# DaDaMrX/ReaLiSe

Measured on AMD Instinct MI355X. Metric: train sentences/sec (seq_len=128), higher is better.
Workload: dtype bf16

## Files before the change

### include/realise_hip_debug.h

```cpp
#ifndef REALISE_HIP_DEBUG_H
#define REALISE_HIP_DEBUG_H
#include "realise_hip.h"
#ifdef __cplusplus
extern "C" {
#endif

void realise_set_tn_transpose_read(int enable);
void realise_set_nt_allow_n96(int on);
void realise_set_nt_variant(int v);
void realise_set_engine(int key, int value);
int realise_gemm_nt_rows(void* stream, int dtype, const void* A, int64_t lda, const void* B, int64_t ldb, int M, int N, int K,
                         const realise_epilogue* ep, const int* rows_dev);
int realise_gemm_nt_live(void* stream, const void* A, int64_t lda, const void* B, int64_t ldb, int M, int N, int K,
                         const realise_epilogue* ep, const int* live_list, const int* live_count);
int realise_gemm_nt_live_rows(void* stream, const void* A, int64_t lda, const void* B, int64_t ldb, int M, int N, int K,
                              const realise_epilogue* ep, const int* row_list, const int* row_count);
int realise_gemm_nt_splitk(void* stream, const void* A, int64_t lda, const void* B, int64_t ldb, int M, int N, int K, int nsplit,
                           float* slab, int64_t slab_stride, const int* m_dev);
int realise_gemm_tn_grouped_live(void* stream, int dtype, int n, const realise_tn_problem* problems, int P, const int* live,
                                 const int* n_live, int list_rows, int overwrite);
int realise_layernorm_bwd_ex(void* stream, const void* dy, const void* xhat, const float* rstd, const float* gamma, void* dx, void* dx_drop,
                             uint32_t drop_seed, uint32_t drop_thresh, float drop_scale, float* dgamma, float* dbeta, float* slots, int rows, int H);
int realise_layernorm_fwd_live(void* stream, const void* x, const float* gamma, const float* beta, float eps, void* y, void* xhat, float* rstd,
                               const uint8_t* row_live, int rows, int H);
int realise_layernorm_bwd_live(void* stream, const void* dy, const void* xhat, const float* rstd, const float* gamma, void* dx, void* dx_drop,
                               uint32_t drop_seed, uint32_t drop_thresh, float drop_scale, float* dgamma, float* dbeta, float* slots,
                               const uint8_t* row_live, int rows, int H);
void realise_set_ln(int key, int value);
int realise_batchnorm_stats_ex(void* stream, const void* x, int P, int C, int hw, const float* counts, int n_stat, const float* gamma, const float* beta,
                               float eps, float momentum, float* running_mean, float* running_var, int64_t* num_batches_tracked, float* mean, float* rstd,
                               float* scale, float* shift, float* sq_scratch, float* slots);
int realise_batchnorm_bwd_ex(void* stream, const void* dy, const void* relu_src, int P, int C, int hw, const float* counts, int n_stat,
                             const void* xa, const float* mean_a, const float* rstd_a, const float* gamma_a, void* dxa, float* dgamma_a, float* dbeta_a,
                             const void* xb, const float* mean_b, const float* rstd_b, const float* gamma_b, void* dxb, float* dgamma_b, float* dbeta_b,
                             float* sums, float* slots);
void realise_set_nt8p(int key, int value);
void realise_set_nt_group_m(int g);
void realise_set_tn_split(int n);
void realise_set_conv_c64(int on);
void realise_set_glyph_dedup(int on);
void realise_set_wgrad_overlap(int on);
void realise_set_branch_overlap(int on);
void realise_set_dgrad_parity(int on);
void realise_set_wgrad_group(int on);

int realise_profile_enable(int max_launches);
void realise_profile_mode(int attached);
void realise_profile_disable(void);
void realise_profile_pause(int paused);
int realise_profile_read(int kernel_family, long long* count, double* total_ms, double* total_work);
int realise_profile_dump(int kernel_family, int max_records, float* ms_out, double* work_out);
// ... 46 lines not shown
```

### realise_amd/_capi.py

```python
import ctypes as C
import os

from .config import MODEL_TYPES

HERE = os.path.dirname(os.path.abspath(__file__))
LIB_PATH = os.path.join(HERE, "librealise_hip.so")

F32, BF16 = 0, 1
F32_BF16X3 = 2
EPI_STORE, EPI_GELU, EPI_DROP_RESID, EPI_GELU_BWD = 0, 1, 2, 4


class GruStep(C.Structure):
    _fields_ = [("n_alive", C.c_int32), ("H", C.c_int32), ("Tp", C.c_int32), ("t", C.c_int32),
                ("table", C.c_void_p), ("pho_idx", C.c_void_p), ("perm", C.c_void_p), ("lens", C.c_void_p),
                ("gh", C.c_void_p), ("b_hh", C.c_void_p), ("h_prev", C.c_void_p), ("h_new", C.c_void_p), ("rzn", C.c_void_p), ("out", C.c_void_p),
                ("dout", C.c_void_p), ("dh", C.c_void_p), ("dgi", C.c_void_p), ("dgh", C.c_void_p), ("onehot", C.c_void_p)]


class Gate(C.Structure):
    _fields_ = [("B", C.c_int32), ("S", C.c_int32), ("H", C.c_int32),
                ("bert", C.c_void_p), ("pho", C.c_void_p), ("res", C.c_void_p), ("masks", C.c_void_p), ("W", C.c_void_p), ("bias", C.c_void_p),
                ("mean", C.c_void_p), ("msum", C.c_void_p), ("g", C.c_void_p), ("fused", C.c_void_p),
                ("dfused", C.c_void_p), ("dbert", C.c_void_p), ("dpho", C.c_void_p), ("dres", C.c_void_p), ("dz", C.c_void_p), ("dW", C.c_void_p),
# ... 68 lines not shown
    "realise_gemm_nt_live": (_I, [_P, _P, _L, _P, _L, _I, _I, _I, C.POINTER(Epilogue), _P, _P]),
    "realise_gemm_nt_live_rows": (_I, [_P, _P, _L, _P, _L, _I, _I, _I, C.POINTER(Epilogue), _P, _P]),
    "realise_gemm_nt_splitk": (_I, [_P, _P, _L, _P, _L, _I, _I, _I, _I, _P, _L, _P]),
    "realise_gemm_tn_grouped_live": (_I, [_P, _I, _I, C.POINTER(TnProblem), _I, _P, _P, _I, _I]),
    "realise_conv_tn": (_I, [_P, _I, _P, _L, C.POINTER(ConvGeom), _I, _I, _I, _P, _P, _L]),
    "realise_set_tn_transpose_read": (None, [_I]),
    "realise_set_nt_allow_n96": (None, [_I]),
    "realise_set_nt_variant": (None, [_I]),
    "realise_set_nt_group_m": (None, [_I]),
    "realise_set_nt8p": (None, [_I, _I]),
    "realise_set_ln": (None, [_I, _I]),
    "realise_set_engine": (None, [_I, _I]),
    "realise_layernorm_bwd_ex": (_I, [_P, _P, _P, _P, _P, _P, _P, C.c_uint32, C.c_uint32, C.c_float, _P, _P, _P, _I, _I]),
    "realise_layernorm_fwd_live": (_I, [_P, _P, _P, _P, C.c_float, _P, _P, _P, _P, _I, _I]),
    "realise_layernorm_bwd_live": (_I, [_P, _P, _P, _P, _P, _P, _P, C.c_uint32, C.c_uint32, C.c_float, _P, _P, _P, _P, _I, _I]),
    "realise_batchnorm_stats_ex": (_I, [_P, _P, _I, _I, _I, _P, _I, _P, _P, C.c_float, C.c_float] + [_P] * 9),
    "realise_batchnorm_bwd_ex": (_I, [_P, _P, _P, _I, _I, _I, _P, _I] + [_P] * 7 + [_P] * 7 + [_P, _P]),
    "realise_debug_bn_plan": (_I, [_I, _I, _I, _I, _I, _I, C.POINTER(BnPlan)]),
    "realise_debug_conv_nt_path": (_I, [_I, C.POINTER(ConvGeom), _L, _I, _I, _I, _I, _I, _I, _I, _L, _L]),
    "realise_conv_nt_ex": (_I, [_P, _I, C.POINTER(ConvGeom), _P, _L, _I, _I, _I, C.POINTER(Epilogue), _P, _I, _P, _L]),
    "realise_conv_dgrad_s2_ex": (_I, [_P, _I, C.POINTER(ConvGeom), _P, _L, _I, C.POINTER(Epilogue), _P]),
    "realise_gemm_nt_ex": (_I, [_P, _I, _P, _L, _P, _L, _I, _I, _I, C.POINTER(Epilogue), _P, _I, _P]),
    "realise_batchnorm_stats_rows": (_I, [_P, _I, _P, _I, _I, _I, _P, _P, _I, _I, _P, _P, _F, _F] + [_P] * 9),
    "realise_batchnorm_apply_rows": (_I, [_P, _I] + [_P] * 7 + [_I, _I, _I, _I, _P]),
    "realise_batchnorm_bwd_rows": (_I, [_P, _I, _P, _P, _I, _I, _I, _P, _P, _I] + [_P] * 7 + [_P] * 7 + [_P, _P]),
    "realise_set_tn_split": (None, [_I]),
    "realise_set_conv_c64": (None, [_I]),
    "realise_set_branch_overlap": (None, [_I]),
    "realise_set_glyph_dedup": (None, [_I]),
    "realise_set_wgrad_overlap": (None, [_I]),
    "realise_set_wgrad_group": (None, [_I]),
    "realise_set_dgrad_parity": (None, [_I]),
    "realise_attention_fwd": (_I, [_P, _I, _P, _P, _P, _L, _P, _P, _L, _P, _I, _I, _I, _U, _U, _F]),
    "realise_attention_bwd": (_I, [_P, _I, _P, _P, _P, _L, _P, _P, _P, _L, _P, _P, _P, _P, _P, _L, _I, _I, _I, _U, _U, _F]),
    "realise_mask_to_additive": (_I, [_P, _P, _P, _I]),
    "realise_layernorm_fwd": (_I, [_P, _I, _P, _P, _P, _F, _P, _P, _P, _I, _I]),
    "realise_layernorm_bwd": (_I, [_P, _I, _P, _P, _P, _P, _P, _P, _P, _I, _I]),
    "realise_layernorm_gelu_bwd": (_I, [_P, _I, _P, _P, _P, _P, _P, _P, _P, _P, _I, _I, _P, _P, _I]),
    "realise_masked_ce": (_I, [_P, _I, _P, _L, _P, _P, _I, _I, _P, _P, _P]),
    "realise_gru_step_fwd": (_I, [_P, _I, C.POINTER(GruStep)]),
    "realise_gru_step_bwd": (_I, [_P, _I, C.POINTER(GruStep)]),
    "realise_gate_fwd": (_I, [_P, _I, C.POINTER(Gate)]),
    "realise_gate_bwd": (_I, [_P, _I, C.POINTER(Gate)]),
    "realise_gate_softmax_fwd": (_I, [_P, _I, C.POINTER(Gate)]),
    "realise_gate_softmax_bwd": (_I, [_P, _I, C.POINTER(Gate)]),
    "realise_sum_fuse_fwd": (_I, [_P, _I, _P, _P, _P, _P, _I, _I]),
    "realise_sum_fuse_bwd": (_I, [_P, _I, _P, _P, _P, _P, _I, _I, _P]),
    "realise_batchnorm_fwd": (_I, [_P, _I, _P, _I, _I, _P, _P, _F, _F, _P, _P, _P, _I, _I, _P, _P, _P, _P]),
    "realise_batchnorm_bwd": (_I, [_P, _I, _P, _P, _P, _P, _P, _P, _I, _I, _P, _P, _P, _P]),
    "realise_embedding_bwd": (_I, [_P, _I, _P, _P, _I, _I, _I, _P, _P, _I, _P]),
    "realise_glyph_unique": (_I, [_P, _P, _I, _I, _P, _P, _P, _P, _P, _P, _I, _P]),
    "realise_segment_sum": (_I, [_P, _I, _P, _P, _I, _I, _P, _P, _P]),
    "realise_layernorm_fwd_chw4": (_I, [_P, _I, _P, _P, _P, _P, _F, _P, _P, _P, _I, _I]),
    "realise_gather_rows_chw4": (_I, [_P, _I, _P, _P, _I, _I, _P]),
    "realise_segment_sum_chw4": (_I, [_P, _I, _P, _P, _I, _I, _P, _P, _P]),
    "realise_argmax": (_I, [_P, _I, _P, _L, _I, _I, _P]),
# ... 126 lines not shown
```

### realise_amd/csrc/capi.hip

```cpp
#include <math.h>
#include <string.h>

#include "attention.h"
#include "engine.h"
#include "gemm.h"
#include "layout.h"
#include "ops.h"
#include "prof.h"
#include "../../include/realise_hip_debug.h"

using namespace rl;
#define RL_TRY(expr) do { const int _rc = (expr); if (_rc != RL_OK) return _rc; } while (0)

struct realise_engine { EngineBase* impl; };

namespace {
#define RL_BY_DTYPE_OR(REFUSED, X3_OK, ...) do { \
    if (dtype == REALISE_BF16) { using E = bf16_t; const int x3 = 0; (void)x3; return (__VA_ARGS__); } \
    if (dtype == REALISE_F32 || ((X3_OK) && dtype == REALISE_F32_BF16X3)) { using E = float; const int x3 = dtype == REALISE_F32_BF16X3; (void)x3; return (__VA_ARGS__); } \
    return (REFUSED); } while (0)
#define RL_BY_DTYPE(X3_OK, ...) RL_BY_DTYPE_OR(RL_ERR_ARG, X3_OK, __VA_ARGS__)

template <typename T> EpiParams<T> to_epi(const realise_epilogue* e, int x3 = 0, const float* col_scale = nullptr, int relu = 0) {
  EpiParams<T> p;
// ... 143 lines not shown
  if (live == nullptr || n_live == nullptr) return RL_ERR_ARG;
  RL_BY_DTYPE(1, tn_grouped<E>((hipStream_t)stream, n, problems, P, x3, live, n_live, list_rows, overwrite));
}
int realise_conv_tn(void* stream, int dtype, const void* A, int64_t lda, const realise_conv_geom* b, int P, int Co, int Ci,
                    float* out, float* scratch, int64_t scratch_elems) {
  return realise_conv_tn_ex(stream, dtype, A, lda, b, P, Co, Ci, out, scratch, scratch_elems, 1.0f, nullptr, nullptr, 0);
}
void realise_set_tn_transpose_read(int enable) { set_tn_transpose_read(enable); }
void realise_set_nt_allow_n96(int on) { set_nt_allow_n96(on); }
void realise_set_nt_variant(int v) { set_nt_variant(v); }
void realise_set_nt_group_m(int g) { set_nt8_group_m(g); }
void realise_set_ln(int key, int value) {
  if (key == 0) set_ln_fast(value); else if (key == 1) set_ln_bwd_blocks(value); else if (key == 2) set_bn_fast(value); else if (key == 3) set_bn_chunks(value); else if (key == 4) set_ce_fast(value); else if (key == 5) set_ln_v2(value); else if (key == 6) set_adamw_reg(value);
}
void realise_set_engine(int key, int value) { if (key == 0) set_fwd_order(value); else if (key >= 1 && key <= 3) set_stream_priority(key - 1, value); else if (key == 4) set_cls_compact(value); else if (key == 5) set_skip_dead(value); else if (key == 6) set_cls_splitk(value); else if (key == 9) set_gru_fuse(value); else if (key == 10) set_live_rows(value); else if (key == 13) set_glyph_fuse(value); else if (key == 14) set_bn_fold(value); else if (key == 15) set_opt_pipe(value); }
void realise_set_nt8p(int key, int value) { if (key == 0) set_nt8p_order(value); else if (key == 1) set_nt8p_wgs(value); else if (key == 3) set_nt8_live_gc(value); }
void realise_set_tn_split(int n) { set_tn_split(n); }
void realise_set_wgrad_group(int on) { set_wgrad_group(on); }
void realise_set_dgrad_parity(int on) { set_dgrad_parity(on); }
void realise_set_conv_c64(int on) { set_conv_c64(on); }
void realise_set_glyph_dedup(int on) { set_glyph_dedup(on); }
void realise_set_wgrad_overlap(int on) { set_wgrad_overlap(on); }
void realise_set_branch_overlap(int on) { set_branch_overlap(on); }

int realise_attention_fwd(void* stream, int dtype, const void* q, const void* k, const void* v, int64_t ldq, const float* mask_add,
                          void* ctx, int64_t ldc, float* lse, int B, int nh, int S, uint32_t drop_seed, uint32_t drop_thresh,
                          float drop_scale) {
  RL_BY_DTYPE(0, attn_fwd<E>((hipStream_t)stream, (const E*)q, (const E*)k, (const E*)v, ldq, mask_add, (E*)ctx, ldc, lse, B, nh, S, drop_seed,
                             drop_thresh, drop_scale));
}
int realise_attention_bwd(void* stream, int dtype, const void* q, const void* k, const void* v, int64_t ldq, const float* mask_add,
// ... 24 lines not shown
                               int saved_rows) {
  if (rows < 0 || saved_rows < 0) return RL_ERR_ARG;
  RL_BY_DTYPE(0, ln_gelu_bwd<E>((hipStream_t)stream, to_ln_gelu_bwd<E>(dy, xhat, rstd, z, gamma, dz, dgamma, dbeta, rows, H, n_rows_dev, row_index,
                                                                        saved_rows)));
}
int realise_layernorm_bwd_ex(void* stream, const void* dy, const void* xhat, const float* rstd, const float* gamma, void* dx, void* dx_drop,
                             uint32_t drop_seed, uint32_t drop_thresh, float drop_scale, float* dgamma, float* dbeta, float* slots, int rows, int H) {
  return realise_layernorm_bwd_live(stream, dy, xhat, rstd, gamma, dx, dx_drop, drop_seed, drop_thresh, drop_scale, dgamma, dbeta, slots, nullptr, rows, H);
}
int realise_layernorm_bwd_live(void* stream, const void* dy, const void* xhat, const float* rstd, const float* gamma, void* dx, void* dx_drop,
                               uint32_t drop_seed, uint32_t drop_thresh, float drop_scale, float* dgamma, float* dbeta, float* slots,
                               const uint8_t* row_live, int rows, int H) {
  return ln_bwd<bf16_t>((hipStream_t)stream, to_ln_bwd<bf16_t>(dy, xhat, rstd, gamma, dx, dgamma, dbeta, rows, H, dx_drop,
                                                               DropParams{drop_seed, drop_thresh, drop_scale}, slots, row_live));
}
int realise_build_pho(void* stream, const int64_t* src_idx, int T, const int64_t* table, const int32_t* vlens, int V, int Tw,
                      int64_t* pho_idx, int32_t* perm, int32_t* lens_sorted, int32_t* n_alive_dev) {
  if (!src_idx || !table || !vlens || !pho_idx || !perm || !lens_sorted || !n_alive_dev) return RL_ERR_ARG;
  return pho_prepare((hipStream_t)stream, src_idx, T, table, vlens, V, Tw, pho_idx, perm, lens_sorted, n_alive_dev);
}
int realise_argmax(void* stream, int dtype, const void* logits, int64_t ld, int rows, int V, int64_t* ids) {
  RL_BY_DTYPE(0, argmax_rows<E>((hipStream_t)stream, (const E*)logits, ld, rows, V, ids));
}
int64_t realise_gemm_nt_decode_scratch_bytes(int dtype, int M, int N, int K, int k) {
  RL_BY_DTYPE_OR(0, 1, nt_decode_scratch_bytes(gemm_nt_decode_path<E>(M, N, K, K, K, k, x3), M, N, k));
}
int realise_gemm_nt_decode(void* stream, int dtype, const void* A, int64_t lda, const void* B, int64_t ldb, int M, int N, int K,
                           const float* bias, const int64_t* labels, const realise_decode* d) {
  if (!d) return RL_ERR_ARG;
  DecodeOut o; o.k = d->k; o.ids = d->ids; o.values = d->values; o.probs = d->probs; o.lse = d->lse; o.label_logit = d->label_logit;
  o.scratch = d->scratch; o.scratch_bytes = d->scratch_bytes;
  RL_BY_DTYPE(1, gemm_nt_decode<E>((hipStream_t)stream, (const E*)A, lda, (const E*)B, ldb, M, N, K, bias, labels, o, x3));
}
int realise_masked_ce(void* stream, int dtype, const void* logits, int64_t ld, const int64_t* labels, const int64_t* loss_mask,
                      int rows, int V, float* loss_out, float* count_scratch, void* dlogits) {
  RL_BY_DTYPE(0, ce_loss<E>((hipStream_t)stream, (const E*)logits, ld, labels, loss_mask, rows, V, loss_out, count_scratch, (E*)dlogits));
}

int realise_gru_step_fwd(void* stream, int dtype, const realise_gru_step* a) {
  if (!a) return RL_ERR_ARG;
  RL_BY_DTYPE(0, gru_step_fwd<E>((hipStream_t)stream, to_gru<E>(a)));
}
int realise_gru_step_bwd(void* stream, int dtype, const realise_gru_step* a) {
  if (!a) return RL_ERR_ARG;
  RL_BY_DTYPE(0, gru_step_bwd<E>((hipStream_t)stream, to_gru<E>(a)));
}
int realise_gate_fwd(void* stream, int dtype, const realise_gate* a) {
  if (!a) return RL_ERR_ARG;
  RL_BY_DTYPE(0, gate_fwd<E>((hipStream_t)stream, to_gate<E>(a)));
}
int realise_gate_bwd(void* stream, int dtype, const realise_gate* a) {
  if (!a) return RL_ERR_ARG;
  RL_BY_DTYPE(0, gate_bwd<E>((hipStream_t)stream, to_gate<E>(a)));
}
int realise_gate_softmax_fwd(void* stream, int dtype, const realise_gate* a) {
  if (!a) return RL_ERR_ARG;
  RL_BY_DTYPE(0, gate_fwd<E>((hipStream_t)stream, to_gate<E>(a, true)));
}
int realise_gate_softmax_bwd(void* stream, int dtype, const realise_gate* a) {
  if (!a) return RL_ERR_ARG;
// ... 289 lines not shown
```

### realise_amd/csrc/gemm.h

```cpp
#pragma once
#include "common.h"

namespace rl {

enum EpiMode {
  EPI_STORE = 0,
  EPI_GELU = 1,
  EPI_DROP_RESID = 2,
  EPI_GELU_BWD = 4,
  EPI_AFFINE = 8,
};

struct DecodeParams {
  int kc = 0;
  int nslab = 0;
  float* rec = nullptr;
  const int64_t* labels = nullptr;
  float* label_logit = nullptr;
};

template <typename T> struct EpiParams {
  int mode = EPI_STORE;
  DecodeParams dec;
  T* out = nullptr;
  int64_t ldo = 0;
  T* out2 = nullptr;
  const float* bias = nullptr;
  const T* aux = nullptr;
  int64_t ldaux = 0;
  float alpha = 1.0f;
  int accumulate = 0;
  uint32_t drop_seed = 0, drop_thresh = 0;
  float drop_scale = 1.0f;
  int rm_hw_shift = -1, rm_w_shift = 0, rm_par = 0;
  int wide = 0;
  const int* m_dev = nullptr;
  int m_exact = 0;
  float* slab = nullptr;
  int64_t slab_stride = 0;
  int ksplit = 1;
  const int* live_list = nullptr;
  const int* live_count = nullptr;
  int live_unit = 16;
  int xcd_gc = 1;
  const float* col_scale = nullptr;
  int relu = 0;
  float* out_f32 = nullptr;
  int64_t ldo_f32 = 0;
  int bias_first = 0;
  const float* gru_table = nullptr;
  const int64_t* gru_pho_idx = nullptr;
  const int* gru_perm = nullptr;
// ... 269 lines not shown
                 const EpiParams<T>& ep);
template <typename T>
int conv_dgrad_s2(hipStream_t st, const ConvLoader<T>& full, const T* B_classes, int64_t ldb, int Cin, const EpiParams<T>& ep);
template <typename T>
int gemm_tn(hipStream_t st, const T* A, int64_t lda, const T* B, int64_t ldb, int P, int I, int J, const TnEpi& ep,
            const int* rows_dev = nullptr);
template <typename T>
int gemm_tn_conv(hipStream_t st, const T* A, int64_t lda, const ConvLoader<T>& lb, int P, int I, int J, const TnEpi& ep);

bool nt8_supported(int M, int N, int K, const EpiParams<bf16_t>& ep, int64_t lda, int64_t ldb);
bool nt8p_supported(int M, int N, int K, const EpiParams<bf16_t>& ep, int64_t lda, int64_t ldb);
int gemm_nt8p(hipStream_t st, const bf16_t* A, int64_t lda, const bf16_t* B, int64_t ldb, int M, int N, int K, const EpiParams<bf16_t>& ep);
void set_nt8p_wgs(int n);
void set_nt8_live_gc(int gc);
void set_nt8p_order(int o);
int gemm_nt8(hipStream_t st, const bf16_t* A, int64_t lda, const bf16_t* B, int64_t ldb, int M, int N, int K,
             const EpiParams<bf16_t>& ep, int tile);
int nt8_tile(int N, int K, int tile);
enum NtPath {
  NT_PATH_REFUSED = -1,
  NT_PATH_NONE = 0,
  NT_PATH_4W_256x64 = 1, NT_PATH_4W_128x128 = 2, NT_PATH_4W_128x96 = 3, NT_PATH_4W_256x128 = 4,
  NT_PATH_8W_256x192 = 5, NT_PATH_8W_128x192 = 6, NT_PATH_8W_128x192Q = 7, NT_PATH_8W_KTAIL = 8,
  NT_PATH_8P = 9, NT_PATH_8P_MDEV = 10,
  NT_PATH_8W_MEXACT = 11,
  NT_PATH_C64 = 12,
};
template <typename T>
int gemm_nt_path(int M, int N, int K, const EpiParams<T>& ep, int64_t lda, int64_t ldb, bool rows_dev);
template <typename T>
// ... 37 lines not shown
```

### realise_amd/csrc/gemm_nt8.hip

```cpp
#include "gemm_dev.h"
#include "nt8_cfg.h"
#include "prof.h"

namespace rl {

static int g_nt8_group_m = 0;
void set_nt8_group_m(int g) { g_nt8_group_m = g; }

__device__ __forceinline__ void tile_coords(int tile, int tiles_n, int ntiles, int group_m, int& tm, int& tn) {
  if (group_m <= 1) { tm = tile / tiles_n; tn = tile - tm * tiles_n; return; }
  const int tiles_m = ntiles / tiles_n;
  const int per_group = group_m * tiles_n;
  const int g = tile / per_group, r = tile - g * per_group;
  const int rows = min(group_m, tiles_m - g * group_m);
  tn = r / rows;
  tm = g * group_m + (r - tn * rows);
}

struct GruRows { int tok[2]; int gi_off[2]; bool ends[2]; uint4 hp[2]; };
template <typename C>
__device__ __forceinline__ void nt8_gru_prefetch(const EpiParams<bf16_t>& ep, GruRows& gr, int mlive, int H, int m0, int tn, int wm, int wn, int lane) {
  const int r = lane >> 2, o = lane & 3;
  const int unit0 = tn * 64 + wn * 32 + o * 8;
#pragma unroll
// ... 63 lines not shown
template <typename C, bool KTAIL = false, int XEPI = 0>
__global__ void __launch_bounds__(512, 2 * C::WGS)
gemm_nt8_kernel(const bf16_t* __restrict__ A_, int64_t lda, const bf16_t* __restrict__ B_, int64_t ldb, int M, int N, int K, int tiles_n,
                int ntiles, int group_m, EpiParams<bf16_t> ep) {
  typedef bf16_t T;
  typedef MmaBF16 Mma;
  constexpr int NPW = C::NPW, NPH = C::NPH, NS = C::NS, LEAD = C::LEAD, SQ = C::SQ, HT = C::HT, MT = C::MT, NT = C::NT;
  extern __shared__ __attribute__((aligned(16))) char smem[];
  const int tid = threadIdx.x, lane = tid & 63, g = lane >> 4, l15 = lane & 15;
  const int wave = __builtin_amdgcn_readfirstlane(tid >> 6);
  const int grp = wave >> 2;
  const int wm = wave / C::WN, wn = wave - wm * C::WN;
  const bf16_t* __restrict__ A = A_;
  const bf16_t* __restrict__ B = B_;
  int tile, split = 0;
  if (!KTAIL && ep.ksplit > 1) {
    const int logical = xcd_remap(blockIdx.x, ntiles * ep.ksplit);
    split = logical / ntiles; tile = logical - split * ntiles;
    const int per = (((K + 63) >> 6) + ep.ksplit - 1) / ep.ksplit;
    const int k0 = split * per * 64;
    A += k0; B += k0; K = min(K - k0, per * 64);
  } else if constexpr (XEPI == 3 || XEPI == 4) {
    tile = 0;
  } else {
    tile = xcd_remap(blockIdx.x, ntiles);
  }
  int tm, tn;
  int nlive = 0;
  constexpr bool LIVE = XEPI == 3 || XEPI == 4;
  constexpr int LUNIT = XEPI == 4 ? 1 : 16;
  if constexpr (LIVE) {
    nlive = *ep.live_count;
    const int tml = (nlive + C::BM / LUNIT - 1) / (C::BM / LUNIT);
    const int ntl = tml * tiles_n;
    if (ep.xcd_gc > 1) {
      const int gc = ep.xcd_gc, gr = 8 / gc, x = blockIdx.x & 7;
      const int j = blockIdx.x >> 3;
      const int rg = x / gc, cg = x - rg * gc, ncl = tiles_n / gc;
      const int r0 = (rg * tml) / gr, r1 = ((rg + 1) * tml) / gr;
      if (j >= (r1 - r0) * ncl) return;
      const int lr = j / ncl;
      tm = r0 + lr; tn = cg * ncl + (j - lr * ncl);
      tile = tm * tiles_n + tn;
    } else {
      if ((int)blockIdx.x >= ntl) return;
      tile = xcd_remap(blockIdx.x, ntl);
      tile_coords(tile, tiles_n, ntl, group_m, tm, tn);
    }
  } else {
    tile_coords(tile, tiles_n, ntiles, group_m, tm, tn);
  }
  const int m0 = tm * C::BM, n0 = tn * C::BN;
  const int mlive = ep.m_dev != nullptr ? *ep.m_dev : M;
  if (!LIVE && m0 >= mlive) return;
  const int mzero = ep.m_exact ? mlive : M;
  GruRows gru_rows;
  if constexpr (XEPI == 2) nt8_gru_prefetch<C>(ep, gru_rows, mlive, N / 3, m0, tn, wave / C::WN, wave % C::WN, lane);
  const int nk = (K + 63) >> 6;
  const int ktail = KTAIL ? (K & 63) : 0;

  const int lrow = lane >> 3;
  const int kchunk_b = (((lane & 7) ^ lrow) << 4);
  int lo[NPW];
  uint32_t go[NPW];
#pragma unroll
  for (int s = 0; s < NPW; ++s) {
    const int p = s * 8 + wave;
    int row, is_b;
// ... 264 lines not shown
template <typename C, bool KTAIL = false, int XEPI = 0>
static int launch_nt8_cfg(hipStream_t st, const bf16_t* A, int64_t lda, const bf16_t* B, int64_t ldb, int M, int N, int K,
                          const EpiParams<bf16_t>& ep) {
  const int tiles_m = (M + C::BM - 1) / C::BM, tiles_n = (N + C::BN - 1) / C::BN, ntiles = tiles_m * tiles_n;
  static bool attr_set = false;
  if (!attr_set) {
    (void)hipFuncSetAttribute((const void*)gemm_nt8_kernel<C, KTAIL, XEPI>, hipFuncAttributeMaxDynamicSharedMemorySize, C::LDS);
    attr_set = true;
  }
  ProfScope ps(st, PK_GEMM_NT, 2.0 * M * N * K);
  if (ep.m_dev != nullptr) prof_set_exec(ep.m_dev, 2.0 * N * K, C::BM, M);
  if constexpr (XEPI == 3) prof_set_exec(ep.live_count, 2.0 * N * K * 16.0, C::BM / 16, M / 16);
  if constexpr (XEPI == 4) prof_set_exec(ep.live_count, 2.0 * N * K, C::BM, M);
  EpiParams<bf16_t> epk = ep;
  epk.bias_first = (N % 4) == 0 && N >= 4;
  int grid = ntiles * (KTAIL || ep.ksplit < 1 ? 1 : ep.ksplit);
  if constexpr (XEPI == 3 || XEPI == 4) { if (ep.xcd_gc > 1) grid = (tiles_m + 8 / ep.xcd_gc) * tiles_n; }
  RL_LAUNCH((gemm_nt8_kernel<C, KTAIL, XEPI>), dim3(grid), dim3(512), C::LDS, st, A, lda, B, ldb, M, N, K, tiles_n, ntiles, g_nt8_group_m, epk);
  return hipGetLastError() == hipSuccess ? RL_OK : RL_ERR_LAUNCH;
}


typedef Nt8Cfg<256, 192, 4, 2, false, 2, 2, 4> Cfg256x192;
typedef Nt8Cfg<128, 192, 2, 4, true, 2, 3, 4> Cfg128x192;
typedef Nt8Cfg<128, 192, 4, 2, false, 2, 2, 4, 2> Cfg128x192q;

bool nt8_supported(int M, int N, int K, const EpiParams<bf16_t>& ep, int64_t lda, int64_t ldb) {
  if (ep.mode == EPI_AFFINE || ep.col_scale != nullptr) return false;
  return (K % 8) == 0 && K >= 64 && (N % 8) == 0 && (ep.ldo % 8) == 0 && (ep.aux == nullptr || (ep.ldaux % 8) == 0) &&
         (lda % 8) == 0 && (ldb % 8) == 0 && M >= 1 && N >= 8 &&
// ... 62 lines not shown
```

### realise_amd/csrc/ops.hip

```cpp
#include "ops.h"

namespace rl {
__global__ void col_fold_kernel(float* __restrict__ slots, int slot_stride, int nrec, int n, float* out0, float* out1, int C, int overwrite, int clean, float alpha);

#define RL_LAUNCH_CHECK() (hipGetLastError() == hipSuccess ? RL_OK : RL_ERR_LAUNCH)
#define RL_TRY(expr) do { const int _rc = (expr); if (_rc != RL_OK) return _rc; } while (0)
static constexpr int LN_MAXV = 4;

__global__ void mask_to_additive_kernel(const int64_t* __restrict__ m, float* __restrict__ out, int n) {
  const int i = blockIdx.x * blockDim.x + threadIdx.x;
  if (i < n) out[i] = (1.0f - (float)m[i]) * -10000.0f;
}
int mask_to_additive(hipStream_t st, const int64_t* masks, float* out, int n) {
  hipLaunchKernelGGL(mask_to_additive_kernel, dim3((n + 255) / 256), dim3(256), 0, st, masks, out, n);
  return RL_LAUNCH_CHECK();
}

template <typename T>
__global__ void __launch_bounds__(256) ln_fwd_kernel(LnFwdArgs<T> a) {
  const int wave = threadIdx.x >> 6, lane = threadIdx.x & 63;
  const int row = blockIdx.x * 4 + wave;
  if (row >= a.rows) return;
  const int H = a.H;
  floatx4 v[LN_MAXV];
// ... 459 lines not shown
    for (int c = threadIdx.x; c < H; c += 256) {
      const float v = red[c] + red[H + c] + red[2 * H + c] + red[3 * H + c];
      if (rec != nullptr) rec[pass * H + c] = v;
      else if (out != nullptr) atomicAdd(out + c, v);
    }
  }
}
typedef __attribute__((ext_vector_type(4))) uint32_t ln_u32x4;
__device__ __forceinline__ void ln_store16(ln_u32x4 v, uint32_t voff, uint32_t soff, __amdgpu_buffer_rsrc_t rsrc) {
#if defined(__HIP_DEVICE_COMPILE__)
  asm volatile("buffer_store_dwordx4 %0, %1, %2, %3 offen\n\ts_nop 1" ::"v"(v), "v"(voff), "s"(rsrc), "s"(soff) : "memory");
#endif
}
struct LnRowA { ln_u32x4 dy[2], xh[2]; };

template <bool DROP>
__global__ void __launch_bounds__(256, 1) ln_bwd16v2_kernel(LnBwdArgs<bf16_t> a) {
  extern __shared__ float ln_lds[];
  const int wave = __builtin_amdgcn_readfirstlane(threadIdx.x >> 6), lane = threadIdx.x & 63;
  const int H = a.H, HH = H >> 1;
  const bool active = lane * 16 < H;
  constexpr uint32_t OOB = 0xFFFFFF00u;
  const uint32_t nbytes = (uint32_t)a.rows * (uint32_t)H * 2u;
  const __amdgpu_buffer_rsrc_t rs_dy = __builtin_amdgcn_make_buffer_rsrc((void*)a.dy, 0, (int)nbytes, 0x00020000);
  const __amdgpu_buffer_rsrc_t rs_xh = __builtin_amdgcn_make_buffer_rsrc((void*)a.xhat, 0, (int)nbytes, 0x00020000);
  const __amdgpu_buffer_rsrc_t rs_dx = __builtin_amdgcn_make_buffer_rsrc((void*)a.dx, 0, (int)nbytes, 0x00020000);
  const __amdgpu_buffer_rsrc_t rs_dd = __builtin_amdgcn_make_buffer_rsrc((void*)(a.dx_drop != nullptr ? a.dx_drop : a.dx), 0, a.dx_drop != nullptr ? (int)nbytes : 0, 0x00020000);
  const int c0 = active ? lane * 8 : 0, c1 = active ? HH + lane * 8 : 0;
  const uint32_t lo0 = active ? (uint32_t)c0 * 2u : OOB, lo1 = active ? (uint32_t)c1 * 2u : OOB;
  const int stride = gridDim.x * 4;
  const int row_first = blockIdx.x * 4 + wave;
// ... 26 lines not shown
#pragma unroll
  for (int i = 0; i < 2; ++i)
#pragma unroll
    for (int j = 0; j < 8; ++j) { dg[i][j] = 0.f; db[i][j] = 0.f; }
  auto process = [&](int k, const LnRowA& r, int keep) {
    const int store = (int)(k < nrow);
    const uint32_t row = (uint32_t)(row_first + k * stride);
    const uint32_t msk = keep ? 0xFFFFFFFFu : 0u;
    const uint32_t row_h = (uint32_t)__builtin_amdgcn_readfirstlane((int)(row * (uint32_t)H));
    float s1 = 0.f, s2 = 0.f;
#pragma unroll
    for (int i = 0; i < 2; ++i) {
      float dy[8], xh[8];
      unpack8(uint4{r.dy[i][0] & msk, r.dy[i][1] & msk, r.dy[i][2] & msk, r.dy[i][3] & msk}, dy);
      unpack8(uint4{r.xh[i][0] & msk, r.xh[i][1] & msk, r.xh[i][2] & msk, r.xh[i][3] & msk}, xh);
#pragma unroll
      for (int j = 0; j < 8; ++j) {
        const float t = dy[j] * gm[i][j];
        s1 += t;
        s2 += t * xh[j];
        dg[i][j] += dy[j] * xh[j];
        db[i][j] += dy[j];
      }
    }
    s1 = wave_sum_dpp(s1) / (float)H;
    s2 = wave_sum_dpp(s2) / (float)H;
    const float rstd = keep ? __builtin_bit_cast(float, __builtin_amdgcn_readlane(__builtin_bit_cast(int, rstd_keep), k & 63)) : 0.f;
    const uint32_t sbase = store ? row * row_bytes : 0u;
    __builtin_amdgcn_sched_barrier(0);
#pragma unroll
    for (int i = 0; i < 2; ++i) {
      if (i) __builtin_amdgcn_sched_barrier(0);
      const int c = i ? c1 : c0;
      float dy[8], xh[8], dx[8];
      unpack8(uint4{r.dy[i][0] & msk, r.dy[i][1] & msk, r.dy[i][2] & msk, r.dy[i][3] & msk}, dy);
      unpack8(uint4{r.xh[i][0] & msk, r.xh[i][1] & msk, r.xh[i][2] & msk, r.xh[i][3] & msk}, xh);
#pragma unroll
      for (int j = 0; j < 8; ++j) dx[j] = rstd * (dy[j] * gm[i][j] - s1 - xh[j] * s2);
      const uint32_t voff = store ? (i ? lo1 : lo0) : OOB;
      ln_store16(__builtin_bit_cast(ln_u32x4, pack8(dx)), voff, sbase, rs_dx);
      if constexpr (DROP) {
#pragma unroll
        for (int hq = 0; hq < 2; ++hq) {
          const floatx4 dm = drop_mult4_nz(a.out_drop.seed, a.out_drop.thresh, a.out_drop.scale, row_h + (uint32_t)(c + 4 * hq));
#pragma unroll
          for (int j = 0; j < 4; ++j) dx[4 * hq + j] *= dm[j];
        }
      }
      ln_store16(__builtin_bit_cast(ln_u32x4, pack8(dx)), voff, sbase, rs_dd);
    }
  };
// ... 76 lines not shown
  if (sites.n > LN_FOLD_MAX || (sites.H & 3)) return RL_ERR_ARG;
  hipLaunchKernelGGL(ln_fold_multi_kernel, dim3((2 * sites.H / 4 + 3) / 4, sites.n), dim3(256), 0, st, sites);
  return RL_LAUNCH_CHECK();
}

template <typename T> int ln_bwd(hipStream_t st, const LnBwdArgs<T>& a) {
  if (a.rows <= 0) return RL_OK;
  if ((a.H & 3) || a.H > LN_MAXV * 256) return RL_ERR_ARG;
  int blocks = (a.rows + 3) / 4;
  const int cap = a.H <= 512 ? 1024 : 768;
  if (blocks > cap) blocks = cap;
  LnBwdArgs<T> b = a;
  if (blocks <= 96 || a.dgamma == nullptr || a.dbeta == nullptr) b.slots = nullptr;
  const int nv = (a.H + 255) / 256;
  if constexpr (sizeof(T) == 2) {
    if (g_ln_fast && a.in_drop.thresh == 0u && (a.H % 16) == 0 && a.H <= 1024 && ((int64_t)a.rows + 8192) * a.H * 2 < (1ll << 32) - 4096) {
      const int groups = (a.rows + 3) / 4;
      if (g_ln_v2) {
        blocks = groups < g_ln_bwd_blocks_v2 ? groups : g_ln_bwd_blocks_v2;
        if (blocks * 256 < a.rows) blocks = (a.rows + 255) / 256;
        if (blocks <= 96 || a.dgamma == nullptr || a.dbeta == nullptr) b.slots = nullptr; else b.slots = a.slots;
        if (b.slots != nullptr && blocks > 1024) return RL_ERR_ARG;
        const size_t lds2 = (size_t)8 * a.H * sizeof(float);
        if (a.out_drop.thresh != 0u) hipLaunchKernelGGL((ln_bwd16v2_kernel<true>), dim3(blocks), dim3(256), lds2, st, b);
        else hipLaunchKernelGGL((ln_bwd16v2_kernel<false>), dim3(blocks), dim3(256), lds2, st, b);
        if (a.deferred_records != nullptr) *a.deferred_records = b.slots != nullptr ? blocks : 0;
        else if (b.slots != nullptr) hipLaunchKernelGGL(ln_fold_kernel, dim3((2 * a.H / 4 + 3) / 4), dim3(256), 0, st, b.slots, blocks, a.H, a.dgamma, a.dbeta);
        return RL_LAUNCH_CHECK();
      }
      blocks = groups < g_ln_bwd_blocks ? groups : g_ln_bwd_blocks;
      if (blocks <= 96 || a.dgamma == nullptr || a.dbeta == nullptr) b.slots = nullptr; else b.slots = a.slots;
      const size_t lds = (size_t)5 * a.H * sizeof(float);
      if (a.out_drop.thresh != 0u) hipLaunchKernelGGL((ln_bwd16_kernel<true>), dim3(blocks), dim3(256), lds, st, b);
      else hipLaunchKernelGGL((ln_bwd16_kernel<false>), dim3(blocks), dim3(256), lds, st, b);
      if (a.deferred_records != nullptr) *a.deferred_records = b.slots != nullptr ? blocks : 0;
      else if (b.slots != nullptr) hipLaunchKernelGGL(ln_fold_kernel, dim3((2 * a.H / 4 + 3) / 4), dim3(256), 0, st, b.slots, blocks, a.H, a.dgamma, a.dbeta);
      return RL_LAUNCH_CHECK();
    }
  }
// ... 1691 lines not shown
```

Baseline: 4215.

## Early-exit dead M-tiles in nt8 GEMM and add input-dropout fast LN backward

The nt8 GEMM now reads the device-side live row count up front and, when enabled (default on), remaps tiles so blocks beyond the live M range exit immediately. This cuts wasted block scheduling when the batch shrinks, for example during GRU steps. The fast v2 LayerNorm backward kernel gains an input-dropout variant, so calls with in_drop can use the fast path instead of falling back to the generic kernel. A fused GRU step entry point and debug/capi bindings are also exposed. Together these mix several unrelated optimizations, and the tile remap changes the block-to-tile mapping.

```diff
diff --git a/include/realise_hip_debug.h b/include/realise_hip_debug.h
--- a/include/realise_hip_debug.h
+++ b/include/realise_hip_debug.h
@@ -26,6 +26,9 @@
 int realise_layernorm_bwd_live(void* stream, const void* dy, const void* xhat, const float* rstd, const float* gamma, void* dx, void* dx_drop,
                                uint32_t drop_seed, uint32_t drop_thresh, float drop_scale, float* dgamma, float* dbeta, float* slots,
                                const uint8_t* row_live, int rows, int H);
+int realise_layernorm_bwd_indrop(void* stream, const void* dy, const void* xhat, const float* rstd, const float* gamma, void* dx,
+                                 uint32_t in_seed, uint32_t in_thresh, float in_scale, float* dgamma, float* dbeta, float* slots,
+                                 const uint8_t* row_live, int rows, int H);
 void realise_set_ln(int key, int value);
 int realise_batchnorm_stats_ex(void* stream, const void* x, int P, int C, int hw, const float* counts, int n_stat, const float* gamma, const float* beta,
                                float eps, float momentum, float* running_mean, float* running_var, int64_t* num_batches_tracked, float* mean, float* rstd,
@@ -35,6 +38,7 @@
                              const void* xb, const float* mean_b, const float* rstd_b, const float* gamma_b, void* dxb, float* dgamma_b, float* dbeta_b,
                              float* sums, float* slots);
 void realise_set_nt8p(int key, int value);
+int realise_gru_step_fused(void* stream, const realise_gru_step* a, const void* w_hh, const int* rows_dev);
 void realise_set_nt_group_m(int g);
 void realise_set_tn_split(int n);
 void realise_set_conv_c64(int on);
diff --git a/realise_amd/_capi.py b/realise_amd/_capi.py
--- a/realise_amd/_capi.py
+++ b/realise_amd/_capi.py
@@ -106,6 +106,7 @@
     "realise_layernorm_bwd_ex": (_I, [_P, _P, _P, _P, _P, _P, _P, C.c_uint32, C.c_uint32, C.c_float, _P, _P, _P, _I, _I]),
     "realise_layernorm_fwd_live": (_I, [_P, _P, _P, _P, C.c_float, _P, _P, _P, _P, _I, _I]),
     "realise_layernorm_bwd_live": (_I, [_P, _P, _P, _P, _P, _P, _P, C.c_uint32, C.c_uint32, C.c_float, _P, _P, _P, _P, _I, _I]),
+    "realise_layernorm_bwd_indrop": (_I, [_P, _P, _P, _P, _P, _P, C.c_uint32, C.c_uint32, C.c_float, _P, _P, _P, _P, _I, _I]),
     "realise_batchnorm_stats_ex": (_I, [_P, _P, _I, _I, _I, _P, _I, _P, _P, C.c_float, C.c_float] + [_P] * 9),
     "realise_batchnorm_bwd_ex": (_I, [_P, _P, _P, _I, _I, _I, _P, _I] + [_P] * 7 + [_P] * 7 + [_P, _P]),
     "realise_debug_bn_plan": (_I, [_I, _I, _I, _I, _I, _I, C.POINTER(BnPlan)]),
@@ -132,6 +133,7 @@
     "realise_masked_ce": (_I, [_P, _I, _P, _L, _P, _P, _I, _I, _P, _P, _P]),
     "realise_gru_step_fwd": (_I, [_P, _I, C.POINTER(GruStep)]),
     "realise_gru_step_bwd": (_I, [_P, _I, C.POINTER(GruStep)]),
+    "realise_gru_step_fused": (_I, [_P, C.POINTER(GruStep), _P, _P]),
     "realise_gate_fwd": (_I, [_P, _I, C.POINTER(Gate)]),
     "realise_gate_bwd": (_I, [_P, _I, C.POINTER(Gate)]),
     "realise_gate_softmax_fwd": (_I, [_P, _I, C.POINTER(Gate)]),
diff --git a/realise_amd/csrc/capi.hip b/realise_amd/csrc/capi.hip
--- a/realise_amd/csrc/capi.hip
+++ b/realise_amd/csrc/capi.hip
@@ -181,7 +181,7 @@
   if (key == 0) set_ln_fast(value); else if (key == 1) set_ln_bwd_blocks(value); else if (key == 2) set_bn_fast(value); else if (key == 3) set_bn_chunks(value); else if (key == 4) set_ce_fast(value); else if (key == 5) set_ln_v2(value); else if (key == 6) set_adamw_reg(value);
 }
 void realise_set_engine(int key, int value) { if (key == 0) set_fwd_order(value); else if (key >= 1 && key <= 3) set_stream_priority(key - 1, value); else if (key == 4) set_cls_compact(value); else if (key == 5) set_skip_dead(value); else if (key == 6) set_cls_splitk(value); else if (key == 9) set_gru_fuse(value); else if (key == 10) set_live_rows(value); else if (key == 13) set_glyph_fuse(value); else if (key == 14) set_bn_fold(value); else if (key == 15) set_opt_pipe(value); }
-void realise_set_nt8p(int key, int value) { if (key == 0) set_nt8p_order(value); else if (key == 1) set_nt8p_wgs(value); else if (key == 3) set_nt8_live_gc(value); }
+void realise_set_nt8p(int key, int value) { if (key == 0) set_nt8p_order(value); else if (key == 1) set_nt8p_wgs(value); else if (key == 3) set_nt8_live_gc(value); else if (key == 4) set_nt8_mdev_split(value); }
 void realise_set_tn_split(int n) { set_tn_split(n); }
 void realise_set_wgrad_group(int on) { set_wgrad_group(on); }
 void realise_set_dgrad_parity(int on) { set_dgrad_parity(on); }
@@ -236,6 +236,13 @@
   return ln_bwd<bf16_t>((hipStream_t)stream, to_ln_bwd<bf16_t>(dy, xhat, rstd, gamma, dx, dgamma, dbeta, rows, H, dx_drop,
                                                                DropParams{drop_seed, drop_thresh, drop_scale}, slots, row_live));
 }
+int realise_layernorm_bwd_indrop(void* stream, const void* dy, const void* xhat, const float* rstd, const float* gamma, void* dx,
+                                 uint32_t in_seed, uint32_t in_thresh, float in_scale, float* dgamma, float* dbeta, float* slots,
+                                 const uint8_t* row_live, int rows, int H) {
+  LnBwdArgs<bf16_t> a = to_ln_bwd<bf16_t>(dy, xhat, rstd, gamma, dx, dgamma, dbeta, rows, H, nullptr, DropParams(), slots, row_live);
+  a.in_drop = DropParams{in_seed, in_thresh, in_scale};
+  return ln_bwd<bf16_t>((hipStream_t)stream, a);
+}
 int realise_build_pho(void* stream, const int64_t* src_idx, int T, const int64_t* table, const int32_t* vlens, int V, int Tw,
                       int64_t* pho_idx, int32_t* perm, int32_t* lens_sorted, int32_t* n_alive_dev) {
   if (!src_idx || !table || !vlens || !pho_idx || !perm || !lens_sorted || !n_alive_dev) return RL_ERR_ARG;
@@ -266,6 +273,14 @@
 int realise_gru_step_bwd(void* stream, int dtype, const realise_gru_step* a) {
   if (!a) return RL_ERR_ARG;
   RL_BY_DTYPE(0, gru_step_bwd<E>((hipStream_t)stream, to_gru<E>(a)));
+}
+int realise_gru_step_fused(void* stream, const realise_gru_step* a, const void* w_hh, const int* rows_dev) {
+  if (!a || !w_hh || !a->h_prev || !a->h_new || !a->out || a->n_alive < 1 || a->H < 64) return RL_ERR_ARG;
+  EpiParams<bf16_t> ep; ep.mode = EPI_STORE; ep.out = (bf16_t*)a->h_new; ep.ldo = a->H; ep.bias = a->b_hh; ep.m_dev = rows_dev;
+  ep.gru_table = a->table; ep.gru_pho_idx = a->pho_idx; ep.gru_perm = a->perm; ep.gru_lens = a->lens;
+  ep.gru_hprev = (const bf16_t*)a->h_prev; ep.gru_rzn = (bf16_t*)a->rzn; ep.gru_gh = (bf16_t*)a->gh; ep.gru_out = (bf16_t*)a->out;
+  ep.gru_Tp = a->Tp; ep.gru_t = a->t;
+  return gemm_nt8_gru((hipStream_t)stream, (const bf16_t*)a->h_prev, a->H, (const bf16_t*)w_hh, a->H, a->n_alive, 3 * a->H, a->H, ep);
 }
 int realise_gate_fwd(void* stream, int dtype, const realise_gate* a) {
   if (!a) return RL_ERR_ARG;
diff --git a/realise_amd/csrc/gemm.h b/realise_amd/csrc/gemm.h
--- a/realise_amd/csrc/gemm.h
+++ b/realise_amd/csrc/gemm.h
@@ -36,6 +36,7 @@
   int wide = 0;
   const int* m_dev = nullptr;
   int m_exact = 0;
+  int mdev_split = 0;
   float* slab = nullptr;
   int64_t slab_stride = 0;
   int ksplit = 1;
@@ -335,6 +336,7 @@
 void set_nt8p_wgs(int n);
 void set_nt8_live_gc(int gc);
 void set_nt8p_order(int o);
+void set_nt8_mdev_split(int on);
 int gemm_nt8(hipStream_t st, const bf16_t* A, int64_t lda, const bf16_t* B, int64_t ldb, int M, int N, int K,
              const EpiParams<bf16_t>& ep, int tile);
 int nt8_tile(int N, int K, int tile);
diff --git a/realise_amd/csrc/gemm_nt8.hip b/realise_amd/csrc/gemm_nt8.hip
--- a/realise_amd/csrc/gemm_nt8.hip
+++ b/realise_amd/csrc/gemm_nt8.hip
@@ -6,6 +6,8 @@
 
 static int g_nt8_group_m = 0;
 void set_nt8_group_m(int g) { g_nt8_group_m = g; }
+static int g_nt8_mdev_split = 1;
+void set_nt8_mdev_split(int on) { g_nt8_mdev_split = on != 0; }
 
 __device__ __forceinline__ void tile_coords(int tile, int tiles_n, int ntiles, int group_m, int& tm, int& tn) {
   if (group_m <= 1) { tm = tile / tiles_n; tn = tile - tm * tiles_n; return; }
@@ -101,25 +103,35 @@
   const bf16_t* __restrict__ A = A_;
   const bf16_t* __restrict__ B = B_;
   int tile, split = 0;
+  constexpr bool LIVE = XEPI == 3 || XEPI == 4;
+  int mlive = M, ntl = ntiles;
+  if constexpr (!LIVE) {
+    if (ep.m_dev != nullptr) {
+      mlive = *ep.m_dev;
+      if (ep.mdev_split) {
+        ntl = min((mlive + C::BM - 1) / C::BM, ntiles / tiles_n) * tiles_n;
+        if ((int)blockIdx.x >= ntl * ((!KTAIL && ep.ksplit > 1) ? ep.ksplit : 1)) return;
+      }
+    }
+  }
   if (!KTAIL && ep.ksplit > 1) {
-    const int logical = xcd_remap(blockIdx.x, ntiles * ep.ksplit);
-    split = logical / ntiles; tile = logical - split * ntiles;
+    const int logical = xcd_remap(blockIdx.x, ntl * ep.ksplit);
+    split = logical / ntl; tile = logical - split * ntl;
     const int per = (((K + 63) >> 6) + ep.ksplit - 1) / ep.ksplit;
     const int k0 = split * per * 64;
     A += k0; B += k0; K = min(K - k0, per * 64);
   } else if constexpr (XEPI == 3 || XEPI == 4) {
     tile = 0;
   } else {
-    tile = xcd_remap(blockIdx.x, ntiles);
+    tile = xcd_remap(blockIdx.x, ntl);
   }
   int tm, tn;
   int nlive = 0;
-  constexpr bool LIVE = XEPI == 3 || XEPI == 4;
   constexpr int LUNIT = XEPI == 4 ? 1 : 16;
   if constexpr (LIVE) {
     nlive = *ep.live_count;
     const int tml = (nlive + C::BM / LUNIT - 1) / (C::BM / LUNIT);
-    const int ntl = tml * tiles_n;
+    ntl = tml * tiles_n;
     if (ep.xcd_gc > 1) {
       const int gc = ep.xcd_gc, gr = 8 / gc, x = blockIdx.x & 7;
       const int j = blockIdx.x >> 3;
@@ -135,10 +147,10 @@
       tile_coords(tile, tiles_n, ntl, group_m, tm, tn);
     }
   } else {
-    tile_coords(tile, tiles_n, ntiles, group_m, tm, tn);
+    tile_coords(tile, tiles_n, ntl, group_m, tm, tn);
   }
   const int m0 = tm * C::BM, n0 = tn * C::BN;
-  const int mlive = ep.m_dev != nullptr ? *ep.m_dev : M;
+  if constexpr (LIVE) mlive = ep.m_dev != nullptr ? *ep.m_dev : M;
   if (!LIVE && m0 >= mlive) return;
   const int mzero = ep.m_exact ? mlive : M;
   GruRows gru_rows;
@@ -433,6 +445,7 @@
   if constexpr (XEPI == 4) prof_set_exec(ep.live_count, 2.0 * N * K, C::BM, M);
   EpiParams<bf16_t> epk = ep;
   epk.bias_first = (N % 4) == 0 && N >= 4;
+  epk.mdev_split = (ep.m_dev != nullptr && g_nt8_mdev_split) ? 1 : 0;
   int grid = ntiles * (KTAIL || ep.ksplit < 1 ? 1 : ep.ksplit);
   if constexpr (XEPI == 3 || XEPI == 4) { if (ep.xcd_gc > 1) grid = (tiles_m + 8 / ep.xcd_gc) * tiles_n; }
   RL_LAUNCH((gemm_nt8_kernel<C, KTAIL, XEPI>), dim3(grid), dim3(512), C::LDS, st, A, lda, B, ldb, M, N, K, tiles_n, ntiles, g_nt8_group_m, epk);
diff --git a/realise_amd/csrc/ops.hip b/realise_amd/csrc/ops.hip
--- a/realise_amd/csrc/ops.hip
+++ b/realise_amd/csrc/ops.hip
@@ -497,7 +497,7 @@
 }
 struct LnRowA { ln_u32x4 dy[2], xh[2]; };
 
-template <bool DROP>
+template <bool DROP, bool IN_DROP = false>
 __global__ void __launch_bounds__(256, 1) ln_bwd16v2_kernel(LnBwdArgs<bf16_t> a) {
   extern __shared__ float ln_lds[];
   const int wave = __builtin_amdgcn_readfirstlane(threadIdx.x >> 6), lane = threadIdx.x & 63;
@@ -554,6 +554,14 @@
       float dy[8], xh[8];
       unpack8(uint4{r.dy[i][0] & msk, r.dy[i][1] & msk, r.dy[i][2] & msk, r.dy[i][3] & msk}, dy);
       unpack8(uint4{r.xh[i][0] & msk, r.xh[i][1] & msk, r.xh[i][2] & msk, r.xh[i][3] & msk}, xh);
+      if constexpr (IN_DROP) {
+#pragma unroll
+        for (int hq = 0; hq < 2; ++hq) {
+          const floatx4 dm = drop_mult4_nz(a.in_drop.seed, a.in_drop.thresh, a.in_drop.scale, row_h + (uint32_t)((i ? c1 : c0) + 4 * hq));
+#pragma unroll
+          for (int j = 0; j < 4; ++j) dy[4 * hq + j] *= dm[j];
+        }
+      }
 #pragma unroll
       for (int j = 0; j < 8; ++j) {
         const float t = dy[j] * gm[i][j];
@@ -575,6 +583,14 @@
       float dy[8], xh[8], dx[8];
       unpack8(uint4{r.dy[i][0] & msk, r.dy[i][1] & msk, r.dy[i][2] & msk, r.dy[i][3] & msk}, dy);
       unpack8(uint4{r.xh[i][0] & msk, r.xh[i][1] & msk, r.xh[i][2] & msk, r.xh[i][3] & msk}, xh);
+      if constexpr (IN_DROP) {
+#pragma unroll
+        for (int hq = 0; hq < 2; ++hq) {
+          const floatx4 dm = drop_mult4_nz(a.in_drop.seed, a.in_drop.thresh, a.in_drop.scale, row_h + (uint32_t)(c + 4 * hq));
+#pragma unroll
+          for (int j = 0; j < 4; ++j) dy[4 * hq + j] *= dm[j];
+        }
+      }
 #pragma unroll
       for (int j = 0; j < 8; ++j) dx[j] = rstd * (dy[j] * gm[i][j] - s1 - xh[j] * s2);
       const uint32_t voff = store ? (i ? lo1 : lo0) : OOB;
@@ -681,7 +697,8 @@
   if (blocks <= 96 || a.dgamma == nullptr || a.dbeta == nullptr) b.slots = nullptr;
   const int nv = (a.H + 255) / 256;
   if constexpr (sizeof(T) == 2) {
-    if (g_ln_fast && a.in_drop.thresh == 0u && (a.H % 16) == 0 && a.H <= 1024 && ((int64_t)a.rows + 8192) * a.H * 2 < (1ll << 32) - 4096) {
+    const bool in_drop_v2 = g_ln_v2 == 1 && a.out_drop.thresh == 0u;
+    if (g_ln_fast && (a.in_drop.thresh == 0u || in_drop_v2) && (a.H % 16) == 0 && a.H <= 1024 && ((int64_t)a.rows + 8192) * a.H * 2 < (1ll << 32) - 4096) {
       const int groups = (a.rows + 3) / 4;
       if (g_ln_v2) {
         blocks = groups < g_ln_bwd_blocks_v2 ? groups : g_ln_bwd_blocks_v2;
@@ -689,7 +706,8 @@
         if (blocks <= 96 || a.dgamma == nullptr || a.dbeta == nullptr) b.slots = nullptr; else b.slots = a.slots;
         if (b.slots != nullptr && blocks > 1024) return RL_ERR_ARG;
         const size_t lds2 = (size_t)8 * a.H * sizeof(float);
-        if (a.out_drop.thresh != 0u) hipLaunchKernelGGL((ln_bwd16v2_kernel<true>), dim3(blocks), dim3(256), lds2, st, b);
+        if (a.in_drop.thresh != 0u) hipLaunchKernelGGL((ln_bwd16v2_kernel<false, true>), dim3(blocks), dim3(256), lds2, st, b);
+        else if (a.out_drop.thresh != 0u) hipLaunchKernelGGL((ln_bwd16v2_kernel<true>), dim3(blocks), dim3(256), lds2, st, b);
         else hipLaunchKernelGGL((ln_bwd16v2_kernel<false>), dim3(blocks), dim3(256), lds2, st, b);
         if (a.deferred_records != nullptr) *a.deferred_records = b.slots != nullptr ? blocks : 0;
         else if (b.slots != nullptr) hipLaunchKernelGGL(ln_fold_kernel, dim3((2 * a.H / 4 + 3) / 4), dim3(256), 0, st, b.slots, blocks, a.H, a.dgamma, a.dbeta);
```

Result: faster. 4310 (median of 5 runs) (+2.2%).
